# LIU-YUXI/SA-GNN

Hardware: AMD Instinct MI355X
Metric: spmm_edges_per_sec (higher is better)
Workload: dtype f32

## Files before the change

### include/sagnn.h

```cpp
#ifndef SAGNN_H
#define SAGNN_H

#include <stddef.h>
#include <stdint.h>

#ifdef __cplusplus
extern "C" {
#endif

#define SAGNN_VERSION 10400

enum {
  SAGNN_OK = 0,
  SAGNN_ERR_NULL = -1,
  SAGNN_ERR_DIM = -2,
  SAGNN_ERR_ALIGN = -3,
  SAGNN_ERR_CSR = -4,
  SAGNN_ERR_ARG = -5,
  SAGNN_ERR_WORKSPACE = -6,
  SAGNN_ERR_NOMEM = -7
};

int sagnn_version(void);

// ... 93 lines not shown
  const sagnn_spmm_plan* adj_user;
  const sagnn_spmm_plan* adj_item;
  const sagnn_spmm_batch* adj_batch;
  void* adj_workspace;
  size_t adj_workspace_bytes;
} sagnn_edge_time;

int sagnn_spmm_time_batch_create(const sagnn_spmm_plan* const* adj_user, const sagnn_spmm_plan* const* adj_item,
                                 int n_intervals, sagnn_spmm_batch** batch_out);

int sagnn_spmm_time_f32(const sagnn_spmm_plan* plan, const float* X, int64_t ldx, int d,
                        const sagnn_spmm_epilogue* epilogue, const sagnn_edge_drop* drop, const sagnn_edge_time* time,
                        void* workspace, size_t workspace_bytes, void* stream);

typedef struct sagnn_gnn_side {
  const float* in;   int64_t ld_in,  slab_in;
  float*       out;  int64_t ld_out, slab_out;
  float*       scratch;
  uint8_t*     mask;
} sagnn_gnn_side;

enum { SAGNN_EDGES_PLAIN = 0, SAGNN_EDGES_DROP = 1, SAGNN_EDGES_TIME = 2 };

typedef struct sagnn_gnn_args {
  sagnn_gnn_side user, item;
  int d, n_layers;
  float leaky;
  int edges;
  const sagnn_edge_drop* drop;
  const sagnn_edge_time* time;
  int interval;
  void* workspace; size_t workspace_bytes;
} sagnn_gnn_args;

int sagnn_gnn_interval_f32(const sagnn_spmm_plan* plan_user, const sagnn_spmm_plan* plan_item, const sagnn_gnn_args* args,
                           void* stream);
int sagnn_gnn_interval_bwd_f32(const sagnn_spmm_plan* plan_user, const sagnn_spmm_plan* plan_item,
                               const sagnn_gnn_args* args, void* stream);
int sagnn_gnn_stack_f32(const sagnn_spmm_batch* batch, const sagnn_gnn_args* args, void* stream);
int sagnn_gnn_stack_bwd_f32(const sagnn_spmm_batch* batch, const sagnn_gnn_args* args, void* stream);

int sagnn_lstm_fwd_f32(const float* x, int64_t ld_n, int64_t ld_t, int64_t n, int t, int d, const float* W,
                       const float* b, float forget_bias, const float* drop_scale, float* h,
                       int64_t ld_h, void* stream);
int sagnn_lstm_fwd_state_f32(const float* x, int64_t ld_n, int64_t ld_t, int64_t n, int t, int d,
                             const float* W, const float* b, float forget_bias, const float* drop_scale,
                             const float* h_init, int64_t ld_hi, const float* c_init, float* h, int64_t ld_h,
                             float* c_final, void* stream);
int sagnn_layernorm_td_f32(const float* x, int64_t ld_n, int64_t ld_t, int64_t n, int t, int d,
                           const float* gamma, const float* beta, float eps, float* y,
                           int64_t ld_y, void* stream);
int sagnn_mhsa_mean_f32(const float* x, int64_t ld_n, int64_t ld_t, int64_t n, int t, int d, int heads,
                        const float* Wq, const float* bq, const float* Wk, const float* bk,
                        const float* Wv, const float* bv, float* out, int64_t ld_out,
                        void* stream);
size_t sagnn_mhsa_wide_workspace_bytes(int64_t n, int t, int d);
int sagnn_mhsa_mean_wide_f32(const float* x, int64_t ld_n, int64_t ld_t, int64_t n, int t, int d, int heads,
                             const float* Wq, const float* bq, const float* Wk, const float* bk, const float* Wv,
                             const float* bv, float* out, int64_t ld_out, void* workspace, size_t workspace_bytes,
                             void* stream);
size_t sagnn_ln_mhsa_mean_workspace_bytes(int64_t n, int t, int d, int heads);
int sagnn_ln_mhsa_mean_f32(const float* x, int64_t ld_n, int64_t ld_t, int64_t n, int t, int d, int heads,
                           const float* ln_gamma, const float* ln_beta, float ln_eps, const float* Wq,
                           const float* bq, const float* Wk, const float* bk, const float* Wv, const float* bv,
                           float* out, int64_t ld_out, void* workspace, size_t workspace_bytes, void* stream);
int sagnn_interval_fusion_f32(const float* x, int64_t ld_n, int64_t ld_t, int64_t n, int t, int d, int heads,
// ... 160 lines not shown
```

### sa-gnn_amd/_lib.py

```python
from __future__ import annotations

import ctypes
import os
from ctypes import POINTER, c_char_p, c_float, c_int, c_int32, c_int64, c_size_t, c_uint32, c_uint64, c_void_p

_HERE = os.path.dirname(os.path.abspath(__file__))
LIB_PATH = os.environ.get("SAGNN_LIB") or os.path.join(_HERE, "lib", "libsagnn.so")


class SagnnError(RuntimeError):
    def __init__(self, code: int, msg: str):
        super().__init__(f"libsagnn error {code}: {msg}")
        self.code = code


class Tuning(ctypes.Structure):
    _fields_ = [("short_thresh", c_int32), ("long_thresh", c_int32), ("chunk_edges", c_int32),
                ("reserved", c_int32)]


class SpmmEpilogue(ctypes.Structure):
    _fields_ = [("leaky", c_float), ("residual", c_void_p), ("ldr", c_int64), ("out", c_void_p),
                ("ldo", c_int64), ("acc_in", c_void_p), ("ld_acc_in", c_int64), ("acc_out", c_void_p),
                ("ld_acc_out", c_int64), ("mask_out", c_void_p), ("mask_in", c_void_p),
# ... 27 lines not shown

class PlanInfo(ctypes.Structure):
    _fields_ = [("n_rows", c_int64), ("n_src", c_int64), ("nnz", c_int64),
                ("n_long_rows", c_int64), ("n_chunks", c_int64), ("short_thresh", c_int32),
                ("long_thresh", c_int32), ("chunk_edges", c_int32), ("max_degree", c_int32),
                ("on_device", c_int32), ("weighted", c_int32)]


SIGNATURES = {
    "sagnn_version": (c_int, []),
    "sagnn_set_engine": (c_int, [c_int]),
    "sagnn_get_engine": (c_int, []),
    "sagnn_range_redo_count": (c_int, [POINTER(c_int64), c_int]),
    "sagnn_last_error": (c_size_t, [c_char_p, c_size_t]),
    "sagnn_profile_enable": (c_int, [c_int]),
    "sagnn_profile_read": (c_int, [c_void_p, c_void_p, c_void_p, c_void_p, c_int, POINTER(c_int)]),
    "sagnn_csr_check_host": (c_int, [c_void_p, c_void_p, c_int64, c_int64, c_int64]),
    "sagnn_spmm_plan_create": (c_int, [c_void_p, c_void_p, c_void_p, c_int64, c_int64, c_int64,
                                       POINTER(Tuning), POINTER(c_void_p)]),
    "sagnn_spmm_plan_destroy": (c_int, [c_void_p]),
    "sagnn_spmm_plan_get_info": (c_int, [c_void_p, POINTER(PlanInfo)]),
    "sagnn_spmm_plan_set_weights": (c_int, [c_void_p, c_void_p]),
    "sagnn_spmm_plan_copy_chunks": (c_int, [c_void_p, c_void_p, c_void_p, c_void_p, c_int64]),
    "sagnn_spmm_workspace_bytes": (c_size_t, [c_void_p, c_int]),
    "sagnn_spmm_f32": (c_int, [c_void_p, c_void_p, c_int64, c_int, c_void_p, c_int64, c_float,
                               c_void_p, c_int64, c_void_p, c_int64, c_void_p, c_int64, c_void_p,
                               c_size_t, c_void_p]),
    "sagnn_spmm_ex_f32": (c_int, [c_void_p, c_void_p, c_int64, c_int, POINTER(SpmmEpilogue), c_void_p, c_size_t,
                                  c_void_p]),
    "sagnn_mask_scale_f32": (c_int, [c_void_p, c_int64, c_void_p, c_float, c_void_p, c_int64, c_int64, c_int, c_void_p]),
    "sagnn_spmm_batch_create": (c_int, [c_void_p, c_void_p, c_int, POINTER(c_void_p)]),
    "sagnn_spmm_batch_destroy": (c_int, [c_void_p]),
    "sagnn_spmm_batch_workspace_bytes": (c_size_t, [c_void_p, c_int]),
    "sagnn_gnn_interval_f32": (c_int, [c_void_p, c_void_p, POINTER(GnnArgs), c_void_p]),
    "sagnn_gnn_interval_bwd_f32": (c_int, [c_void_p, c_void_p, POINTER(GnnArgs), c_void_p]),
    "sagnn_gnn_stack_f32": (c_int, [c_void_p, POINTER(GnnArgs), c_void_p]),
    "sagnn_gnn_stack_bwd_f32": (c_int, [c_void_p, POINTER(GnnArgs), c_void_p]),
    "sagnn_spmm_drop_f32": (c_int, [c_void_p, c_void_p, c_int64, c_int, POINTER(SpmmEpilogue), POINTER(EdgeDropArgs),
                                    c_uint32, c_int, c_void_p, c_size_t, c_void_p]),
    "sagnn_spmm_plan_set_buckets": (c_int, [c_void_p, c_void_p, c_int32]),
    "sagnn_spmm_time_batch_create": (c_int, [c_void_p, c_void_p, c_int, POINTER(c_void_p)]),
    "sagnn_spmm_time_f32": (c_int, [c_void_p, c_void_p, c_int64, c_int, POINTER(SpmmEpilogue), POINTER(EdgeDropArgs),
                                    POINTER(EdgeTimeArgs), c_void_p, c_size_t, c_void_p]),
    "sagnn_lstm_fwd_train_f32": (c_int, [c_void_p, c_int64, c_int64, c_int64, c_int, c_int, c_void_p, c_void_p, c_float,
                                         c_void_p, c_void_p, c_int64, c_void_p, c_void_p, c_void_p]),
    "sagnn_mhsa_wide_workspace_bytes": (c_size_t, [c_int64, c_int, c_int]),
    "sagnn_ln_mhsa_mean_workspace_bytes": (c_size_t, [c_int64, c_int, c_int, c_int]),
    "sagnn_ln_mhsa_mean_f32": (c_int, [c_void_p, c_int64, c_int64, c_int64, c_int, c_int, c_int, c_void_p, c_void_p,
                                       c_float, c_void_p, c_void_p, c_void_p, c_void_p, c_void_p, c_void_p, c_void_p,
                                       c_int64, c_void_p, c_size_t, c_void_p]),
    "sagnn_mhsa_mean_wide_f32": (c_int, [c_void_p, c_int64, c_int64, c_int64, c_int, c_int, c_int, c_void_p, c_void_p,
                                         c_void_p, c_void_p, c_void_p, c_void_p, c_void_p, c_int64, c_void_p, c_size_t,
                                         c_void_p]),
    "sagnn_attn_bwd_f32": (c_int, [c_void_p, c_void_p, c_int64, c_int64, c_int, c_int, c_int, c_void_p]),
    "sagnn_layernorm_td_bwd_f32": (c_int, [c_void_p, c_int64, c_void_p, c_int64, c_int64, c_int, c_int, c_void_p,
                                           c_float, c_void_p, c_int64, c_void_p, c_void_p, c_void_p]),
    "sagnn_lstm_bwd_step_f32": (c_int, [c_void_p, c_void_p, c_void_p, c_int64, c_void_p, c_void_p, c_int64, c_void_p,
                                        c_void_p, c_void_p, c_int64, c_int, c_int, c_int, c_void_p]),
    "sagnn_attn_bwd_front_supported": (c_int, [c_int, c_int, c_int]),
    "sagnn_attn_bwd_front_f32": (c_int, [c_void_p, c_int64, c_int64, c_int64, c_int, c_int, c_int, c_void_p, c_void_p,
                                         c_float, c_int, c_void_p, c_void_p, c_void_p, c_void_p, c_void_p, c_void_p,
                                         c_void_p, c_int64, c_void_p, c_void_p, c_void_p]),
    "sagnn_attn_bwd_tail_supported": (c_int, [c_int]),
    "sagnn_attn_bwd_tail_f32": (c_int, [c_void_p, c_void_p, c_int64, c_int, c_void_p, c_void_p, c_void_p, c_void_p]),
    "sagnn_lstm_bwd_supported": (c_int, [c_int]),
    "sagnn_lstm_bwd_f32": (c_int, [c_void_p, c_int64, c_int64, c_void_p, c_void_p, c_void_p, c_void_p, c_int64, c_void_p,
# ... 130 lines not shown
```

### sa-gnn_amd/csrc/spmm.hip

```cpp
#include <float.h>

#include <algorithm>
#include <new>
#include <type_traits>
#include <vector>

#include "common.h"
#include "philox.h"

namespace {

constexpr int kWave = 64;
constexpr int kBlock = 256;
constexpr int kWavesPerBlock = kBlock / kWave;
constexpr int kRowsPerWave = 16;
constexpr int64_t kSmallRows = 262144;
constexpr int kUnroll = 8;

struct Epilogue {
  const float* residual;
  int64_t ldr;
  const float* acc_in;
  int64_t ld_acc_in;
  float* out;
// ... 362 lines not shown
          else cw[u] = 1.f;
          if constexpr (TIME) cb[u] = __shfl(bk, grp * LPR + j + u);
          else cb[u] = 0;
        }
#pragma unroll
        for (int u = 0; u < kUnroll; ++u) {
          v[u] = make_float4(0.f, 0.f, 0.f, 0.f);
          if (c[u] >= 0 && lane_on) v[u] = ld4(X + (int64_t)c[u] * ldx + col);
        }
        if constexpr (TIME) {
#pragma unroll
          for (int u = 0; u < kUnroll; ++u)
            if (c[u] >= 0 && lane_on) add4(v[u], ld4(tm.te + cb[u] * d + col));
        }
#pragma unroll
        for (int u = 0; u < kUnroll; ++u) acc4<WEIGHTED>(acc, cw[u], v[u]);
      }
    }
    if (mine && lane_on) finish_row(ep, row0 + lr, col, drop_scale<DROP>(dr, acc));
  }

  while (medium) {
    const int lr = __builtin_ctzll(medium);
    medium &= medium - 1;
    const int e0 = __builtin_amdgcn_readlane(rp, lr);
    const int dg = __builtin_amdgcn_readlane(deg_l, lr);
    const float4 s =
        wave_row_sum<LPR, false, DROP, WEIGHTED, TIME>(colidx, e0, e0 + dg, X, ldx, lane, grp, col, lane_on, dr, (int)row0 + lr, w,
                                                       tm, d);
    if (grp == 0 && lane_on) finish_row(ep, row0 + lr, col, drop_scale<DROP>(dr, s));
  }
}

template <int LPR, int RPW, class... DropArgs>
__global__ __launch_bounds__(kBlock) void spmm_rows_kernel(
    const int32_t* __restrict__ rowptr, const int32_t* __restrict__ colidx,
    const float* __restrict__ X, int64_t ldx, int d, int64_t n_rows, int short_t, int long_t,
    const int32_t* __restrict__ chunk_e0, const int32_t* __restrict__ chunk_e1, int64_t n_chunks,
    int chunk_blocks, float* __restrict__ partial, Epilogue ep, typename KernelArg<DropArgs>::type... da) {
  constexpr bool DROP = Pack<DropArgs...>::DROP, WEIGHTED = Pack<DropArgs...>::WEIGHTED, TIME = Pack<DropArgs...>::TIME;
  const int lane = threadIdx.x & (kWave - 1);
  const int wave = threadIdx.x / kWave;

  if ((int)blockIdx.x < chunk_blocks) {
    const int grp = lane / LPR;
    const int col = 4 * (lane % LPR);
    const bool lane_on = col < d;
    const int64_t ci = (int64_t)blockIdx.x * kWavesPerBlock + wave;
    if (ci >= n_chunks) return;
    const float4 s = wave_row_sum<LPR, false, DROP, WEIGHTED, TIME>(
        colidx, chunk_e0[ci], chunk_e1[ci], X, ldx, lane, grp, col, lane_on, arg_of<RowDrop, DropArgs...>(da...),
        chunk_row_of<DropArgs...>(ci, da...), weights_of<DropArgs...>(0, da...), arg_of<RowTime, DropArgs...>(da...), d);
    if (grp == 0 && lane_on) st4(partial + ci * (int64_t)d + col, s);
    return;
  }

  const int64_t row0 = ((int64_t)(blockIdx.x - chunk_blocks) * kWavesPerBlock + wave) * RPW;
  if (row0 >= n_rows) return;
  rows_wave<LPR, RPW, DROP, WEIGHTED, TIME>(rowptr, colidx, X, ldx, d, n_rows, row0, short_t, long_t, ep, lane,
                                            arg_of<RowDrop, DropArgs...>(da...), weights_of<DropArgs...>(0, da...),
                                            arg_of<RowTime, DropArgs...>(da...));
}

template <int LPR, class... Scale>
__global__ __launch_bounds__(kBlock) void spmm_fixup_kernel(const int32_t* __restrict__ long_row,
                                                           const int32_t* __restrict__ long_slot,
                                                           int64_t n_long,
                                                           const float* __restrict__ partial, int d,
                                                           Epilogue ep, Scale... scale) {
  static_assert(sizeof...(Scale) <= 1, "drop-only argument: none, or the scale");
  const int lane = threadIdx.x & (kWave - 1);
  const int wave = threadIdx.x / kWave;
  const int grp = lane / LPR;
  const int col = 4 * (lane % LPR);
  const bool lane_on = col < d;
  const int64_t li = (int64_t)blockIdx.x * kWavesPerBlock + wave;
  if (li >= n_long) return;
  const float4 s = wave_row_sum<LPR, true>(nullptr, long_slot[li], long_slot[li + 1], partial, d,
                                           lane, grp, col, lane_on);
  if (grp == 0 && lane_on) finish_row(ep, long_row[li], col, scaled(s, scale...));
}

struct SegMeta {
  const int32_t* rowptr;
  const int32_t* colidx;
  int32_t short_t, long_t;
};
struct DirArgs {
  const float* X;
  int64_t ldx, s_X;
  Epilogue ep;
  int64_t s_res, s_acc_in, s_out, s_acc_out, s_mask_out, s_mask_in, s_out2, s_acc_in2;
};
struct BatchGeom {
  int32_t T;
  int32_t chunk_blocks;
  int32_t blocks_u, blocks_i;
  int32_t rows_u, rows_i;
};

__device__ __forceinline__ Epilogue seg_epilogue(const DirArgs& a, int k) {
  Epilogue e = a.ep;
  if (e.residual) e.residual += (int64_t)k * a.s_res;
  if (e.acc_in) e.acc_in += (int64_t)k * a.s_acc_in;
  if (e.out) e.out += (int64_t)k * a.s_out;
  if (e.acc_out) e.acc_out += (int64_t)k * a.s_acc_out;
  if (e.mask_out) e.mask_out += (int64_t)k * a.s_mask_out;
  if (e.mask_in) e.mask_in += (int64_t)k * a.s_mask_in;
  if (e.out2) e.out2 += (int64_t)k * a.s_out2;
  if (e.acc_in2) e.acc_in2 += (int64_t)k * a.s_acc_in2;
  return e;
}

// ... 228 lines not shown
    return sagnn::fail(SAGNN_ERR_ALIGN, "buckets: pointer must be 2-byte aligned");
  plan->d_buckets = d_buckets;
  plan->n_buckets = d_buckets ? n_buckets : 0;
  return SAGNN_OK;
}

extern "C" int sagnn_spmm_plan_get_info(const sagnn_spmm_plan* plan, sagnn_spmm_plan_info* info) {
  if (!plan || !info) return sagnn::fail(SAGNN_ERR_NULL, "plan/info is NULL");
  *info = plan->info;
  return SAGNN_OK;
}

extern "C" int sagnn_spmm_plan_copy_chunks(const sagnn_spmm_plan* plan, int32_t* rows,
                                           int32_t* e_begin, int32_t* e_end, int64_t cap) {
  if (!plan) return sagnn::fail(SAGNN_ERR_NULL, "plan is NULL");
  const int64_t n = plan->info.n_chunks;
  if (cap < n) return sagnn::fail(SAGNN_ERR_ARG, "cap %lld < n_chunks %lld", (long long)cap, (long long)n);
  if (n > 0 && (!rows || !e_begin || !e_end)) return sagnn::fail(SAGNN_ERR_NULL, "null output array");
  std::copy(plan->chunk_row.begin(), plan->chunk_row.end(), rows);
  std::copy(plan->chunk_e0.begin(), plan->chunk_e0.end(), e_begin);
  std::copy(plan->chunk_e1.begin(), plan->chunk_e1.end(), e_end);
  return SAGNN_OK;
}

extern "C" size_t sagnn_spmm_workspace_bytes(const sagnn_spmm_plan* plan, int d) {
  if (!plan || d <= 0) return 0;
  return (size_t)plan->info.n_chunks * (size_t)d * sizeof(float);
}

namespace {

template <int LPR>
int launch_spmm(const sagnn_spmm_plan* p, const float* X, int64_t ldx, int d, const Epilogue& ep,
                float* partial, hipStream_t stream, const RowDrop* drop = nullptr, const float* te = nullptr) {
  const int64_t n_rows = p->info.n_rows;
  const int64_t n_chunks = p->info.n_chunks;
  const int64_t chunk_blocks = (n_chunks + kWavesPerBlock - 1) / kWavesPerBlock;
  constexpr int G = kWave / LPR;
  constexpr int RPW_SMALL = G > 4 ? G : 4;
  const bool small = n_rows < kSmallRows;
  const int64_t rows_per_block = (int64_t)kWavesPerBlock * (small ? RPW_SMALL : kRowsPerWave);
  const int64_t row_blocks = (n_rows + rows_per_block - 1) / rows_per_block;
  const int64_t blocks = chunk_blocks + row_blocks;
  if (blocks > INT32_MAX) return sagnn::fail(SAGNN_ERR_ARG, "grid too large");
  if (blocks > 0) {
    sagnn::ProfileScope prof(sagnn::kProfSpmmRows, stream, p->info.nnz, n_rows);
    const auto rows = [&](auto kernel, auto... da) {
      hipLaunchKernelGGL(kernel, dim3((unsigned)blocks), dim3(kBlock), 0, stream, p->d_rowptr, p->d_colidx, X, ldx, d, n_rows,
                         p->info.short_thresh, p->info.long_thresh, p->d_chunk_e0, p->d_chunk_e1, n_chunks,
                         (int)chunk_blocks, partial, ep, da...);
    };
    const float* w = p->d_weights;
    const RowTime tm{p->d_buckets, te};
    if (te && w)
      rows(small ? spmm_rows_kernel<LPR, RPW_SMALL, RowTime, const float*> : spmm_rows_kernel<LPR, kRowsPerWave, RowTime, const float*>,
           tm, w);
    else if (te)
      rows(small ? spmm_rows_kernel<LPR, RPW_SMALL, RowTime> : spmm_rows_kernel<LPR, kRowsPerWave, RowTime>, tm);
    else if (drop && w)
      rows(small ? spmm_rows_kernel<LPR, RPW_SMALL, const int32_t*, RowDrop, const float*>
                 : spmm_rows_kernel<LPR, kRowsPerWave, const int32_t*, RowDrop, const float*>,
           p->d_chunk_row, *drop, w);
    else if (drop)
      rows(small ? spmm_rows_kernel<LPR, RPW_SMALL, const int32_t*, RowDrop> : spmm_rows_kernel<LPR, kRowsPerWave, const int32_t*, RowDrop>,
           p->d_chunk_row, *drop);
    else if (w)
      rows(small ? spmm_rows_kernel<LPR, RPW_SMALL, const float*> : spmm_rows_kernel<LPR, kRowsPerWave, const float*>, w);
    else
      rows(small ? spmm_rows_kernel<LPR, RPW_SMALL> : spmm_rows_kernel<LPR, kRowsPerWave>);
    SAGNN_HIP_TRY(hipGetLastError());
  }
  const int64_t n_long = p->info.n_long_rows;
  if (n_long > 0) {
    sagnn::ProfileScope prof(sagnn::kProfSpmmFixup, stream, n_chunks, n_long);
    const int64_t fb = (n_long + kWavesPerBlock - 1) / kWavesPerBlock;
    const auto fixup = [&](auto kernel, auto... scale) {
      hipLaunchKernelGGL(kernel, dim3((unsigned)fb), dim3(kBlock), 0, stream,
                         p->d_long_row, p->d_long_slot, n_long, partial, d, ep, scale...);
    };
    if (drop) fixup(spmm_fixup_kernel<LPR, float>, drop->scale);
    else fixup(spmm_fixup_kernel<LPR>);
    SAGNN_HIP_TRY(hipGetLastError());
  }
  return SAGNN_OK;
}

int check_mat(const char* name, const void* ptr, int64_t ld, int d, bool required) {
  if (!ptr) return required ? sagnn::fail(SAGNN_ERR_NULL, "%s is NULL", name) : SAGNN_OK;
  if (!sagnn::aligned16(ptr) || (ld & 3) != 0)
    return sagnn::fail(SAGNN_ERR_ALIGN, "%s: pointer must be 16-byte aligned and ld a multiple of 4", name);
  if (ld < d) return sagnn::fail(SAGNN_ERR_ARG, "%s: ld %lld < d %d", name, (long long)ld, d);
  return SAGNN_OK;
}

int check_d(int d) {
  if (d < 4 || d > 256 || (d & 3)) return sagnn::fail(SAGNN_ERR_DIM, "d = %d: need a multiple of 4 in [4, 256]", d);
  return SAGNN_OK;
}

struct Slab {
  float* p;
  int64_t ld, slab;
};

int check_slab(const char* name, const Slab& x, int d) {
  if (int rc = check_mat(name, x.p, x.ld, d, true)) return rc;
  if (x.slab & 3) return sagnn::fail(SAGNN_ERR_ALIGN, "%s: slab stride must be a multiple of 4", name);
  return SAGNN_OK;
}

int launch_mask_scale(const Slab& g, const uint8_t* mask, int64_t s_mask, float slope, const Slab& out, int64_t n_rows,
                      int d, int64_t T, hipStream_t stream) {
  const int64_t n = n_rows * (d / 4);
  if (n == 0) return SAGNN_OK;
  hipLaunchKernelGGL(mask_scale_kernel, dim3((unsigned)((n + 255) / 256), (unsigned)T), dim3(256), 0, stream, g.p, g.ld,
                     g.slab, mask, s_mask, d / 4, slope, out.p, out.ld, out.slab, n_rows, d);
  SAGNN_HIP_TRY(hipGetLastError());
  return SAGNN_OK;
}

Epilogue kernel_epilogue(const sagnn_spmm_epilogue& e, int d) {
  return Epilogue{e.residual, e.ldr,      e.acc_in,  e.ld_acc_in, e.out,  e.ldo,    e.acc_out, e.ld_acc_out,
                  e.leaky,    e.mask_out, e.mask_in, e.out2,      e.ldo2, e.slope2, d / 4,     e.acc_in2,
                  e.ld_acc_in2};
}

int spmm_ex(const sagnn_spmm_plan* plan, const float* X, int64_t ldx, int d, const Epilogue& e, void* workspace,
            size_t workspace_bytes, void* stream, const RowDrop* drop = nullptr, const float* te = nullptr) {
  if (!plan->info.on_device) return sagnn::fail(SAGNN_ERR_ARG, "plan was built host-only (no device CSR)");
  if (int rc = check_d(d)) return rc;
  if (te) {
    if (drop) return sagnn::fail(SAGNN_ERR_ARG, "edge time: no product takes a drop and a time term");
    if (!plan->d_buckets) return sagnn::fail(SAGNN_ERR_ARG, "edge time: the plan has no buckets (sagnn_spmm_plan_set_buckets)");
    if (!sagnn::aligned16(te)) return sagnn::fail(SAGNN_ERR_ALIGN, "edge time: TE must be 16-byte aligned");
  }
  if (!e.out && !e.acc_out && !e.out2) return sagnn::fail(SAGNN_ERR_NULL, "no output given");
  if (int rc = check_mat("X", X, ldx, d, plan->info.nnz > 0)) return rc;
  if (int rc = check_mat("residual", e.residual, e.ldr, d, false)) return rc;
  if (int rc = check_mat("out", e.out, e.ldo, d, false)) return rc;
  if (int rc = check_mat("acc_in", e.acc_in, e.ld_acc_in, d, false)) return rc;
  if (int rc = check_mat("acc_out", e.acc_out, e.ld_acc_out, d, false)) return rc;
  if (int rc = check_mat("acc_in2", e.acc_in2, e.ld_acc_in2, d, false)) return rc;
  if (e.acc_in2 && !e.acc_out) return sagnn::fail(SAGNN_ERR_ARG, "acc_in2 given without acc_out");
  if (int rc = check_mat("out2", e.out2, e.ldo2, d, false)) return rc;
  if ((e.out && e.out == X) || (e.acc_out && e.acc_out == X) || (e.out2 && e.out2 == X))
    return sagnn::fail(SAGNN_ERR_ARG, "outputs must not alias X");
  if (e.mask_in && !e.out2) return sagnn::fail(SAGNN_ERR_ARG, "mask_in given without out2");
  const size_t need = sagnn_spmm_workspace_bytes(plan, d);
  if (need > 0) {
    if (!workspace || workspace_bytes < need)
      return sagnn::fail(SAGNN_ERR_WORKSPACE, "workspace needs %zu bytes, got %zu", need,
                         workspace ? workspace_bytes : (size_t)0);
    if (!sagnn::aligned16(workspace)) return sagnn::fail(SAGNN_ERR_ALIGN, "workspace not 16-byte aligned");
  }
  if (plan->info.n_rows == 0) return SAGNN_OK;

  hipStream_t s = static_cast<hipStream_t>(stream);
  float* partial = static_cast<float*>(workspace);
  switch (sagnn::lanes_per_row(d)) {
    case 8: return launch_spmm<8>(plan, X, ldx, d, e, partial, s, drop, te);
    case 16: return launch_spmm<16>(plan, X, ldx, d, e, partial, s, drop, te);
    case 32: return launch_spmm<32>(plan, X, ldx, d, e, partial, s, drop, te);
    default: return launch_spmm<64>(plan, X, ldx, d, e, partial, s, drop, te);
  }
}

}

extern "C" int sagnn_spmm_ex_f32(const sagnn_spmm_plan* plan, const float* X, int64_t ldx, int d,
                                 const sagnn_spmm_epilogue* e, void* workspace, size_t workspace_bytes,
                                 void* stream) {
  if (!plan || !e) return sagnn::fail(SAGNN_ERR_NULL, "plan/epilogue is NULL");
  return spmm_ex(plan, X, ldx, d, kernel_epilogue(*e, d), workspace, workspace_bytes, stream);
}

namespace {
constexpr int kDropMaxLayers = 127;
constexpr int64_t kDropMaxIntervals = 1 << 23;

int check_drop(const sagnn_edge_drop* drop, int n_layers, int64_t last_interval) {
  if (!drop) return sagnn::fail(SAGNN_ERR_NULL, "edge drop: the sagnn_edge_drop is NULL");
  if (drop->keep_threshold == 0) return sagnn::fail(SAGNN_ERR_ARG, "edge drop: keep_threshold = 0 keeps no edge");
  if (!(drop->scale > 0.f) || !(drop->scale <= FLT_MAX))
    return sagnn::fail(SAGNN_ERR_ARG, "edge drop: scale = %g, need a finite value > 0", (double)drop->scale);
  if (n_layers > kDropMaxLayers)
    return sagnn::fail(SAGNN_ERR_ARG, "edge drop: n_layers = %d, the tag holds %d", n_layers, kDropMaxLayers);
  if (last_interval < 0 || last_interval >= kDropMaxIntervals)
    return sagnn::fail(SAGNN_ERR_ARG, "edge drop: interval %lld outside [0, 2^23)", (long long)last_interval);
  return SAGNN_OK;
}

RowDrop row_drop(const sagnn_edge_drop& e, uint32_t tag, bool rows_users) {
  return RowDrop{(uint32_t)e.seed, (uint32_t)(e.seed >> 32), e.step, e.keep_threshold, tag, rows_users ? 1 : 0, e.scale};
}
}

extern "C" int sagnn_spmm_drop_f32(const sagnn_spmm_plan* plan, const float* X, int64_t ldx, int d,
// ... 368 lines not shown
  int operator()(int, const Slab&, const Slab&) const { return SAGNN_OK; }
};
template <class Launch, class BeforeStep = NoBeforeStep>
int run_backward(const Stack& st, Launch launch, void* stream, BeforeStep before_step = BeforeStep{}) {
  for (const Side* s : {&st.u, &st.i}) {
    const int64_t mrow = st.d / 4;
    if (int rc = launch_mask_scale(s->in, s->mask + (int64_t)(st.n_layers - 1) * s->rows * mrow, st.n_layers * s->rows * mrow,
                                   st.leaky, scratch_slot(st, *s, 2), s->rows, st.d, st.T, static_cast<hipStream_t>(stream)))
      return rc;
  }
  for (int l = st.n_layers - 1; l >= 0; --l) {
    const int cur = (st.n_layers - 1 - l) & 1;
    if (int rc = before_step(l, scratch_slot(st, st.u, 2 + cur), scratch_slot(st, st.i, 2 + cur))) return rc;
    if (int rc = launch(backward_step(st, st.u, st.i, l), backward_step(st, st.i, st.u, l),
                        LayerTags{(uint32_t)l << 1 | 1u, (uint32_t)l << 1, l}))
      return rc;
  }
  return SAGNN_OK;
}

auto batched(const sagnn_spmm_batch* b, int d, void* workspace, void* stream) {
  return [=](const DirArgs& au, const DirArgs& ai, const LayerTags&) {
    return launch_batch_d(b, d, au, ai, static_cast<float*>(workspace), static_cast<hipStream_t>(stream));
  };
}

auto batched_drop(const sagnn_spmm_batch* b, int d, void* workspace, void* stream, const sagnn_edge_drop& drop) {
  return [=](const DirArgs& au, const DirArgs& ai, const LayerTags& t) {
    const BatchDrop bd{row_drop(drop, t.tag_u, true), t.tag_i};
    return launch_batch_d(b, d, au, ai, static_cast<float*>(workspace), static_cast<hipStream_t>(stream), &bd);
  };
}

auto per_plan(const sagnn_spmm_plan* plan_user, const sagnn_spmm_plan* plan_item, int d, void* workspace,
              size_t workspace_bytes, void* stream) {
  return [=](const DirArgs& au, const DirArgs& ai, const LayerTags&) {
    if (int rc = spmm_ex(plan_user, au.X, au.ldx, d, au.ep, workspace, workspace_bytes, stream)) return rc;
    return spmm_ex(plan_item, ai.X, ai.ldx, d, ai.ep, workspace, workspace_bytes, stream);
  };
}

auto per_plan_drop(const sagnn_spmm_plan* plan_user, const sagnn_spmm_plan* plan_item, int d, void* workspace,
                   size_t workspace_bytes, void* stream, const sagnn_edge_drop& drop, int interval) {
  return [=](const DirArgs& au, const DirArgs& ai, const LayerTags& t) {
    const uint32_t k = (uint32_t)interval << 8;
    const RowDrop du = row_drop(drop, t.tag_u | k, true), di = row_drop(drop, t.tag_i | k, false);
    if (int rc = spmm_ex(plan_user, au.X, au.ldx, d, au.ep, workspace, workspace_bytes, stream, &du)) return rc;
    return spmm_ex(plan_item, ai.X, ai.ldx, d, ai.ep, workspace, workspace_bytes, stream, &di);
  };
}

int check_time(const sagnn_edge_time* t, const sagnn_edge_drop* drop, int32_t n_buckets, int d) {
  if (drop) return sagnn::fail(SAGNN_ERR_ARG, "edge time: edge dropout and time do not combine (drop must be NULL)");
  if (!t || !t->te) return sagnn::fail(SAGNN_ERR_NULL, "edge time: the sagnn_edge_time or its te is NULL");
  if (n_buckets == 0) return sagnn::fail(SAGNN_ERR_ARG, "edge time: the plans carry no buckets (sagnn_spmm_plan_set_buckets)");
  if (t->n_buckets != n_buckets)
    return sagnn::fail(SAGNN_ERR_ARG, "edge time: n_buckets = %d but the plans were given %d", t->n_buckets, n_buckets);
  if (!sagnn::aligned16(t->te) || ((t->stride_interval | t->stride_layer | t->stride_dir) & 3) || (d & 3))
    return sagnn::fail(SAGNN_ERR_ALIGN, "edge time: te must be 16-byte aligned and its strides multiples of 4");
  return SAGNN_OK;
}

int check_time_bwd(const sagnn_edge_time* t, bool stack, int64_t U, int64_t I, int T) {
  if (!t->dte) return sagnn::fail(SAGNN_ERR_NULL, "edge time: dte is NULL");
  if (!sagnn::aligned16(t->dte)) return sagnn::fail(SAGNN_ERR_ALIGN, "edge time: dte must be 16-byte aligned");
  if (stack) {
    const sagnn_spmm_batch* b = t->adj_batch;
    if (!b) return sagnn::fail(SAGNN_ERR_NULL, "edge time: adj_batch is NULL");
    if (b->T != T || b->U != t->n_buckets || b->I != t->n_buckets)
      return sagnn::fail(SAGNN_ERR_ARG, "edge time: adj_batch is not the time batch of %d intervals and %d buckets", T, t->n_buckets);
    return SAGNN_OK;
// ... 120 lines not shown
  if (int rc = check_form(g, a, false)) return rc;
  if (int rc = check_graphs(g)) return rc;
  const sagnn_gnn_side &u = a->user, &i = a->item;
  if (!u.in || !i.in || !u.out || !i.out) return sagnn::fail(SAGNN_ERR_NULL, "null embedding pointer");
  if (g.stack)
    if (int rc = check_d(a->d)) return rc;
  if (a->n_layers < 1) return sagnn::fail(SAGNN_ERR_ARG, "n_layers = %d: need >= 1", a->n_layers);
  if ((u.mask == nullptr) != (i.mask == nullptr)) return sagnn::fail(SAGNN_ERR_NULL, "give both masks or neither");
  if (a->n_layers > 1 && (!u.scratch || !i.scratch))
    return sagnn::fail(SAGNN_ERR_NULL, "scratch buffers required for n_layers > 1");
  if (!g.stack) {
    if (!g.plan_user->info.on_device) return sagnn::fail(SAGNN_ERR_ARG, "plan was built host-only (no device CSR)");
    if (int rc = check_d(a->d)) return rc;
  }
  const Stack st = make_stack(g, *a);
  if (int rc = check_stack(st, a->n_layers > 1, "u0", "i0", "user_out", "item_out")) return rc;
  if (g.stack)
    if (int rc = check_batch_ws(g.batch, a->d, a->workspace, a->workspace_bytes)) return rc;
  return with_launcher(g, *a, stream, [&](auto launch) { return run_forward(st, launch); });
}

int gnn_backward(const Graphs& g, const sagnn_gnn_args* a, void* stream) {
  if (int rc = check_form(g, a, true)) return rc;
  if (int rc = check_graphs(g)) return rc;
  const sagnn_gnn_side &u = a->user, &i = a->item;
  if (!u.in || !i.in || !u.out || !i.out || !u.mask || !i.mask || !u.scratch || !i.scratch)
    return sagnn::fail(SAGNN_ERR_NULL, "null pointer");
  if (a->n_layers < 1) return sagnn::fail(SAGNN_ERR_ARG, "n_layers = %d: need >= 1", a->n_layers);
  if (int rc = check_d(a->d)) return rc;
  const Stack st = make_stack(g, *a);
  if (int rc = check_stack(st, true, "G_u", "G_i", "grad_u0", "grad_i0")) return rc;
  if (g.stack)
    if (int rc = check_batch_ws(g.batch, a->d, a->workspace, a->workspace_bytes)) return rc;
  if (a->edges != SAGNN_EDGES_TIME)
    return with_launcher(g, *a, stream, [&](auto launch) { return run_backward(st, launch, stream); });
  const sagnn_edge_time& tm = *a->time;
  if (!g.stack)
    return run_backward(st, per_plan(g.plan_user, g.plan_item, a->d, a->workspace, a->workspace_bytes, stream), stream,
                        dte_per_plan(tm, a->d, a->interval, stream));
  if (int rc = check_batch_ws(tm.adj_batch, a->d, tm.adj_workspace, tm.adj_workspace_bytes)) return rc;
  return run_backward(st, batched(g.batch, a->d, a->workspace, stream), stream, dte_batched(tm, a->d, stream));
}
}

extern "C" int sagnn_gnn_interval_f32(const sagnn_spmm_plan* plan_user, const sagnn_spmm_plan* plan_item,
                                      const sagnn_gnn_args* args, void* stream) {
  return gnn_forward(Graphs{plan_user, plan_item, nullptr, false}, args, stream);
}

extern "C" int sagnn_gnn_interval_bwd_f32(const sagnn_spmm_plan* plan_user, const sagnn_spmm_plan* plan_item,
                                          const sagnn_gnn_args* args, void* stream) {
  return gnn_backward(Graphs{plan_user, plan_item, nullptr, false}, args, stream);
}

extern "C" int sagnn_gnn_stack_f32(const sagnn_spmm_batch* batch, const sagnn_gnn_args* args, void* stream) {
  return gnn_forward(Graphs{nullptr, nullptr, batch, true}, args, stream);
}

extern "C" int sagnn_gnn_stack_bwd_f32(const sagnn_spmm_batch* batch, const sagnn_gnn_args* args, void* stream) {
  return gnn_backward(Graphs{nullptr, nullptr, batch, true}, args, stream);
}

extern "C" int sagnn_spmm_time_f32(const sagnn_spmm_plan* plan, const float* X, int64_t ldx, int d,
                                   const sagnn_spmm_epilogue* e, const sagnn_edge_drop* drop, const sagnn_edge_time* time,
                                   void* workspace, size_t workspace_bytes, void* stream) {
  if (!plan || !e) return sagnn::fail(SAGNN_ERR_NULL, "plan/epilogue is NULL");
  if (int rc = check_time(time, drop, plan->n_buckets, d)) return rc;
  return spmm_ex(plan, X, ldx, d, kernel_epilogue(*e, d), workspace, workspace_bytes, stream, nullptr, time->te);
}
```

### sa-gnn_amd/ops.py

```python
from __future__ import annotations

import ctypes
import math

import numpy as np
import torch

from . import _lib
from ._lib import PlanInfo, Tuning, check

SUPPORTED_D = tuple(range(4, 257, 4))

ENGINES = {"f16x2": 0, "f32": 1, "valu": 2}


def set_engine(name: str) -> None:
    check(_lib.load().sagnn_set_engine(ENGINES[name]))


def get_engine() -> str:
    code = _lib.load().sagnn_get_engine()
    return next(k for k, v in ENGINES.items() if v == code)


# ... 122 lines not shown
        w_t = None if weights is None else _check_weights(weights, self.nnz)
        if w_t is not None and device is None:
            raise ValueError("weights: a host-only plan (device=None) takes no weights")
        if (buckets is None) != (n_buckets is None):
            raise ValueError("buckets: give buckets and n_buckets together")
        b_t = None if buckets is None else _check_buckets(buckets, n_buckets, self.nnz)
        if b_t is not None and device is None:
            raise ValueError("buckets: a host-only plan (device=None) takes no buckets")
        rp_h = rp_t.cpu().contiguous()
        self._rowptr_host = rp_h.numpy()
        if validate:
            ci_h = ci_t.cpu().contiguous()
            check(lib.sagnn_csr_check_host(rp_h.data_ptr(), ci_h.data_ptr(), self.n_rows, self.n_src,
                                           self.nnz))
        tun = None
        if tuning is not None:
            tun = Tuning(int(tuning[0]), int(tuning[1]), int(tuning[2]), 0)
        if device is None:
            self.rowptr = self.colidx = None
            d_rp = d_ci = None
        else:
            self.rowptr = rp_t.to(device).contiguous()
            self.colidx = ci_t.to(device).contiguous()
            if self.colidx.numel() == 0:
                self.colidx = torch.zeros(1, dtype=torch.int32, device=device)
            d_rp, d_ci = self.rowptr.data_ptr(), self.colidx.data_ptr()
        check(lib.sagnn_spmm_plan_create(rp_h.data_ptr(), d_rp, d_ci, self.n_rows, self.n_src,
                                         self.nnz, ctypes.byref(tun) if tun else None,
                                         ctypes.byref(self._h)))
        info = PlanInfo()
        check(lib.sagnn_spmm_plan_get_info(self._h, ctypes.byref(info)))
        self.info = info
        self.device = device
        self._ws: dict[int, torch.Tensor] = {}
        self.partner_adjoint: SpmmPlan | None = None
        self.weights = None
        if w_t is not None:
            self.weights = w_t.to(device).contiguous()
            if self.weights.numel() == 0:
                self.weights = torch.zeros(1, dtype=torch.float32, device=device)
            check(lib.sagnn_spmm_plan_set_weights(self._h, self.weights.data_ptr()))
            check(lib.sagnn_spmm_plan_get_info(self._h, ctypes.byref(info)))
        self.buckets, self.n_buckets = None, 0
        self._tuning = tuning
        self._time_adjoint: SpmmPlan | None = None
        if b_t is not None:
            self._buckets_host = b_t.numpy()
            self._weights_host = None if w_t is None else w_t.numpy()
            self.n_buckets = int(n_buckets)
            self.buckets = b_t.to(device).contiguous()
            if self.buckets.numel() == 0:
                self.buckets = torch.zeros(1, dtype=torch.uint16, device=device)
            check(lib.sagnn_spmm_plan_set_buckets(self._h, self.buckets.data_ptr(), self.n_buckets))

    @property
    def time_adjoint(self) -> "SpmmPlan":
        if self.buckets is None:
            raise ValueError("time_adjoint: the plan has no buckets")
        if self._time_adjoint is None:
            rp, ci, w = time_adjoint_arrays(self._rowptr_host, self._buckets_host, self.n_buckets, self._weights_host)
            self._time_adjoint = SpmmPlan(rp, ci, self.n_buckets, self.n_rows, device=self.device, tuning=self._tuning,
                                          validate=False, weights=w)
        return self._time_adjoint

    @property
    def weighted(self) -> bool:
        return self.weights is not None
# ... 143 lines not shown
        a.stride_layer = te.stride(-4)
        a.stride_interval = te.stride(0) if stack else 0
        self.keep = [te, dte, adj]
        if dte is not None:
            a.dte = dte.data_ptr()
            if stack:
                a.adj_batch = adj.handle
                ws = adj.workspace(d)
            else:
                a.adj_user, a.adj_item = adj[0].handle, adj[1].handle
                ws = _interval_ws(adj[0], adj[1], d)
            self.keep.append(ws)
            a.adj_workspace, a.adj_workspace_bytes = _ptr(ws), 0 if ws is None else ws.numel() * 4
        self.args = a


def spmm_time(plan: SpmmPlan, x: torch.Tensor | None, leaky: float, te: torch.Tensor, residual=None, out=None, acc_in=None,
              acc_out=None, acc_in2=None, mask_out=None, mask_in=None, out2=None, slope2: float = 1.0,
              want_out: bool = False):
    if plan.buckets is None:
        raise ValueError("spmm_time: the plan has no buckets (SpmmPlan(..., buckets=, n_buckets=))")
    return spmm_ex(plan, x, leaky, residual, out, acc_in, acc_out, acc_in2, mask_out, mask_in, out2, slope2, want_out,
                   _time=te)


def mask_scale(g: torch.Tensor, mask: torch.Tensor, slope: float, out: torch.Tensor):
    rows, d = int(g.shape[0]), int(g.shape[1])
    _masks("mask", mask, (rows, d // 4))
    check(_lib.load().sagnn_mask_scale_f32(_ptr(g), _f32_rows("g", g, d, rows), _ptr(mask), float(slope), _ptr(out),
                                           _f32_rows("out", out, d, rows), rows, d, _stream()))
    return out


def _interval_ws(plan_user: SpmmPlan, plan_item: SpmmPlan, d: int):
    wu, wi = plan_user.workspace(d), plan_item.workspace(d)
    return wu if (wi is None or (wu is not None and wu.numel() >= wi.numel())) else wi


def _scratch(name: str, s: torch.Tensor | None, k: int, rows: int, d: int, device):
    if s is None:
        return torch.empty(k * rows * d, dtype=torch.float32, device=device)
    if s.dtype != torch.float32 or not s.is_contiguous() or s.numel() < k * rows * d:
        raise ValueError(f"{name}: need a contiguous float32 buffer of {k}*{rows}*{d} elements")
    return s


def _masks(name: str, m: torch.Tensor, shape: tuple):
    if m.dtype != torch.uint8 or not m.is_contiguous() or m.numel() != int(np.prod(shape)):
        raise ValueError(f"{name}: need a contiguous uint8 tensor {list(shape)}")
    return m


def _adjoint_pair(plan_user: SpmmPlan, plan_item: SpmmPlan):
    adj_u, adj_i = plan_user.partner_adjoint, plan_item.partner_adjoint
    if (adj_u is None) != (adj_i is None):
        raise ValueError("give the exact adjoint of both plans or of neither")
    if adj_u is not None:
        return adj_u, adj_i
    if plan_user.nnz != plan_item.nnz:
        raise ValueError(f"plans are not a transposed pair (nnz {plan_user.nnz} vs {plan_item.nnz}: duplicated stored "
                         "entries?) — build them with graph.interval_pair, which adds the exact adjoints")
    return plan_user, plan_item


def _gnn_args(user: tuple, item: tuple, d: int, n_layers: int, leaky: float, drop, interval: int, et, ws):
    if et is not None and drop is not None:
        raise ValueError("edge dropout and time do not combine: give `drop` or `time`, not both")
    a = _lib.GnnArgs()
    for side, (x, ld_in, slab_in, out, ld_out, slab_out, scratch, mask) in ((a.user, user), (a.item, item)):
# ... 1186 lines not shown
```

Before: 17.65 billion.

## Fold first side's long-row fixup into second side's SpMM launch

In the interval GNN forward, the two per-side SpMM calls now use separate workspace regions. The long-row fixup of the first side runs as extra guest blocks at the front of the second side's rows kernel instead of as its own launch. This removes one kernel launch and its serialization per layer, and orders the side with more chunks first. The cost is a larger combined workspace, a new workspace check, and a dispatch branch at the start of every plain SpMM kernel block.

```diff
diff --git a/include/sagnn.h b/include/sagnn.h
--- a/include/sagnn.h
+++ b/include/sagnn.h
@@ -149,6 +149,9 @@
   int interval;
   void* workspace; size_t workspace_bytes;
 } sagnn_gnn_args;
+
+size_t sagnn_gnn_interval_workspace_bytes(const sagnn_spmm_plan* plan_user, const sagnn_spmm_plan* plan_item, int d);
+int sagnn_gnn_interval_first_side(const sagnn_spmm_plan* plan_user, const sagnn_spmm_plan* plan_item);
 
 int sagnn_gnn_interval_f32(const sagnn_spmm_plan* plan_user, const sagnn_spmm_plan* plan_item, const sagnn_gnn_args* args,
                            void* stream);
diff --git a/sa-gnn_amd/_lib.py b/sa-gnn_amd/_lib.py
--- a/sa-gnn_amd/_lib.py
+++ b/sa-gnn_amd/_lib.py
@@ -83,6 +83,8 @@
     "sagnn_spmm_batch_create": (c_int, [c_void_p, c_void_p, c_int, POINTER(c_void_p)]),
     "sagnn_spmm_batch_destroy": (c_int, [c_void_p]),
     "sagnn_spmm_batch_workspace_bytes": (c_size_t, [c_void_p, c_int]),
+    "sagnn_gnn_interval_workspace_bytes": (c_size_t, [c_void_p, c_void_p, c_int]),
+    "sagnn_gnn_interval_first_side": (c_int, [c_void_p, c_void_p]),
     "sagnn_gnn_interval_f32": (c_int, [c_void_p, c_void_p, POINTER(GnnArgs), c_void_p]),
     "sagnn_gnn_interval_bwd_f32": (c_int, [c_void_p, c_void_p, POINTER(GnnArgs), c_void_p]),
     "sagnn_gnn_stack_f32": (c_int, [c_void_p, POINTER(GnnArgs), c_void_p]),
diff --git a/sa-gnn_amd/csrc/spmm.hip b/sa-gnn_amd/csrc/spmm.hip
--- a/sa-gnn_amd/csrc/spmm.hip
+++ b/sa-gnn_amd/csrc/spmm.hip
@@ -418,21 +418,56 @@
   }
 }
 
+template <int LPR, class... Scale>
+__device__ __forceinline__ void fixup_wave(const int32_t* __restrict__ long_row, const int32_t* __restrict__ long_slot,
+                                           int64_t n_long, const float* __restrict__ partial, int d, const Epilogue& ep,
+                                           int block, Scale... scale) {
+  static_assert(sizeof...(Scale) <= 1, "drop-only argument: none, or the scale");
+  const int lane = threadIdx.x & (kWave - 1);
+  const int wave = threadIdx.x / kWave;
+  const int grp = lane / LPR;
+  const int col = 4 * (lane % LPR);
+  const bool lane_on = col < d;
+  const int64_t li = (int64_t)block * kWavesPerBlock + wave;
+  if (li >= n_long) return;
+  const float4 s = wave_row_sum<LPR, true>(nullptr, long_slot[li], long_slot[li + 1], partial, d,
+                                           lane, grp, col, lane_on);
+  if (grp == 0 && lane_on) finish_row(ep, long_row[li], col, scaled(s, scale...));
+}
+
+struct Guest {
+  const int32_t* long_row;
+  const int32_t* long_slot;
+  const float* partial;
+  int64_t n_long;
+  int blocks;
+  int d;
+  Epilogue ep;
+};
+
 template <int LPR, int RPW, class... DropArgs>
 __global__ __launch_bounds__(kBlock) void spmm_rows_kernel(
     const int32_t* __restrict__ rowptr, const int32_t* __restrict__ colidx,
     const float* __restrict__ X, int64_t ldx, int d, int64_t n_rows, int short_t, int long_t,
     const int32_t* __restrict__ chunk_e0, const int32_t* __restrict__ chunk_e1, int64_t n_chunks,
-    int chunk_blocks, float* __restrict__ partial, Epilogue ep, typename KernelArg<DropArgs>::type... da) {
+    int chunk_blocks, float* __restrict__ partial, Epilogue ep, Guest guest, typename KernelArg<DropArgs>::type... da) {
   constexpr bool DROP = Pack<DropArgs...>::DROP, WEIGHTED = Pack<DropArgs...>::WEIGHTED, TIME = Pack<DropArgs...>::TIME;
+  int block = (int)blockIdx.x;
+  if constexpr (!DROP && !TIME) {
+    if (block < guest.blocks) {
+      fixup_wave<LPR>(guest.long_row, guest.long_slot, guest.n_long, guest.partial, guest.d, guest.ep, block);
+      return;
+    }
+    block -= guest.blocks;
+  }
   const int lane = threadIdx.x & (kWave - 1);
   const int wave = threadIdx.x / kWave;
 
-  if ((int)blockIdx.x < chunk_blocks) {
+  if (block < chunk_blocks) {
     const int grp = lane / LPR;
     const int col = 4 * (lane % LPR);
     const bool lane_on = col < d;
-    const int64_t ci = (int64_t)blockIdx.x * kWavesPerBlock + wave;
+    const int64_t ci = (int64_t)block * kWavesPerBlock + wave;
     if (ci >= n_chunks) return;
     const float4 s = wave_row_sum<LPR, false, DROP, WEIGHTED, TIME>(
         colidx, chunk_e0[ci], chunk_e1[ci], X, ldx, lane, grp, col, lane_on, arg_of<RowDrop, DropArgs...>(da...),
@@ -441,7 +476,7 @@
     return;
   }
 
-  const int64_t row0 = ((int64_t)(blockIdx.x - chunk_blocks) * kWavesPerBlock + wave) * RPW;
+  const int64_t row0 = ((int64_t)(block - chunk_blocks) * kWavesPerBlock + wave) * RPW;
   if (row0 >= n_rows) return;
   rows_wave<LPR, RPW, DROP, WEIGHTED, TIME>(rowptr, colidx, X, ldx, d, n_rows, row0, short_t, long_t, ep, lane,
                                             arg_of<RowDrop, DropArgs...>(da...), weights_of<DropArgs...>(0, da...),
@@ -454,17 +489,7 @@
                                                            int64_t n_long,
                                                            const float* __restrict__ partial, int d,
                                                            Epilogue ep, Scale... scale) {
-  static_assert(sizeof...(Scale) <= 1, "drop-only argument: none, or the scale");
-  const int lane = threadIdx.x & (kWave - 1);
-  const int wave = threadIdx.x / kWave;
-  const int grp = lane / LPR;
-  const int col = 4 * (lane % LPR);
-  const bool lane_on = col < d;
-  const int64_t li = (int64_t)blockIdx.x * kWavesPerBlock + wave;
-  if (li >= n_long) return;
-  const float4 s = wave_row_sum<LPR, true>(nullptr, long_slot[li], long_slot[li + 1], partial, d,
-                                           lane, grp, col, lane_on);
-  if (grp == 0 && lane_on) finish_row(ep, long_row[li], col, scaled(s, scale...));
+  fixup_wave<LPR>(long_row, long_slot, n_long, partial, d, ep, (int)blockIdx.x, scale...);
 }
 
 struct SegMeta {
@@ -759,7 +784,8 @@
 
 template <int LPR>
 int launch_spmm(const sagnn_spmm_plan* p, const float* X, int64_t ldx, int d, const Epilogue& ep,
-                float* partial, hipStream_t stream, const RowDrop* drop = nullptr, const float* te = nullptr) {
+                float* partial, hipStream_t stream, const RowDrop* drop = nullptr, const float* te = nullptr,
+                const Guest* guest = nullptr, bool own_fixup = true) {
   const int64_t n_rows = p->info.n_rows;
   const int64_t n_chunks = p->info.n_chunks;
   const int64_t chunk_blocks = (n_chunks + kWavesPerBlock - 1) / kWavesPerBlock;
@@ -768,14 +794,16 @@
   const bool small = n_rows < kSmallRows;
   const int64_t rows_per_block = (int64_t)kWavesPerBlock * (small ? RPW_SMALL : kRowsPerWave);
   const int64_t row_blocks = (n_rows + rows_per_block - 1) / rows_per_block;
-  const int64_t blocks = chunk_blocks + row_blocks;
+  if (guest && (drop || te)) return sagnn::fail(SAGNN_ERR_ARG, "a drop or time launch carries no guest fix-up");
+  const Guest gst = guest ? *guest : Guest{};
+  const int64_t blocks = gst.blocks + chunk_blocks + row_blocks;
   if (blocks > INT32_MAX) return sagnn::fail(SAGNN_ERR_ARG, "grid too large");
   if (blocks > 0) {
     sagnn::ProfileScope prof(sagnn::kProfSpmmRows, stream, p->info.nnz, n_rows);
     const auto rows = [&](auto kernel, auto... da) {
       hipLaunchKernelGGL(kernel, dim3((unsigned)blocks), dim3(kBlock), 0, stream, p->d_rowptr, p->d_colidx, X, ldx, d, n_rows,
                          p->info.short_thresh, p->info.long_thresh, p->d_chunk_e0, p->d_chunk_e1, n_chunks,
-                         (int)chunk_blocks, partial, ep, da...);
+                         (int)chunk_blocks, partial, ep, gst, da...);
     };
     const float* w = p->d_weights;
     const RowTime tm{p->d_buckets, te};
@@ -798,7 +826,7 @@
     SAGNN_HIP_TRY(hipGetLastError());
   }
   const int64_t n_long = p->info.n_long_rows;
-  if (n_long > 0) {
+  if (n_long > 0 && own_fixup) {
     sagnn::ProfileScope prof(sagnn::kProfSpmmFixup, stream, n_chunks, n_long);
     const int64_t fb = (n_long + kWavesPerBlock - 1) / kWavesPerBlock;
     const auto fixup = [&](auto kernel, auto... scale) {
@@ -852,8 +880,8 @@
                   e.ld_acc_in2};
 }
 
-int spmm_ex(const sagnn_spmm_plan* plan, const float* X, int64_t ldx, int d, const Epilogue& e, void* workspace,
-            size_t workspace_bytes, void* stream, const RowDrop* drop = nullptr, const float* te = nullptr) {
+int spmm_check(const sagnn_spmm_plan* plan, const float* X, int64_t ldx, int d, const Epilogue& e, const void* workspace,
+               size_t workspace_bytes, const RowDrop* drop = nullptr, const float* te = nullptr) {
   if (!plan->info.on_device) return sagnn::fail(SAGNN_ERR_ARG, "plan was built host-only (no device CSR)");
   if (int rc = check_d(d)) return rc;
   if (te) {
@@ -880,16 +908,27 @@
                          workspace ? workspace_bytes : (size_t)0);
     if (!sagnn::aligned16(workspace)) return sagnn::fail(SAGNN_ERR_ALIGN, "workspace not 16-byte aligned");
   }
+  return SAGNN_OK;
+}
+
+int spmm_launch(const sagnn_spmm_plan* plan, const float* X, int64_t ldx, int d, const Epilogue& e, void* workspace,
+                void* stream, const RowDrop* drop = nullptr, const float* te = nullptr, const Guest* guest = nullptr,
+                bool own_fixup = true) {
   if (plan->info.n_rows == 0) return SAGNN_OK;
-
   hipStream_t s = static_cast<hipStream_t>(stream);
   float* partial = static_cast<float*>(workspace);
   switch (sagnn::lanes_per_row(d)) {
-    case 8: return launch_spmm<8>(plan, X, ldx, d, e, partial, s, drop, te);
-    case 16: return launch_spmm<16>(plan, X, ldx, d, e, partial, s, drop, te);
-    case 32: return launch_spmm<32>(plan, X, ldx, d, e, partial, s, drop, te);
-    default: return launch_spmm<64>(plan, X, ldx, d, e, partial, s, drop, te);
-  }
+    case 8: return launch_spmm<8>(plan, X, ldx, d, e, partial, s, drop, te, guest, own_fixup);
+    case 16: return launch_spmm<16>(plan, X, ldx, d, e, partial, s, drop, te, guest, own_fixup);
+    case 32: return launch_spmm<32>(plan, X, ldx, d, e, partial, s, drop, te, guest, own_fixup);
+    default: return launch_spmm<64>(plan, X, ldx, d, e, partial, s, drop, te, guest, own_fixup);
+  }
+}
+
+int spmm_ex(const sagnn_spmm_plan* plan, const float* X, int64_t ldx, int d, const Epilogue& e, void* workspace,
+            size_t workspace_bytes, void* stream, const RowDrop* drop = nullptr, const float* te = nullptr) {
+  if (int rc = spmm_check(plan, X, ldx, d, e, workspace, workspace_bytes, drop, te)) return rc;
+  return spmm_launch(plan, X, ldx, d, e, workspace, stream, drop, te);
 }
 
 }
@@ -1324,11 +1363,29 @@
   };
 }
 
+bool item_side_first(const sagnn_spmm_plan* plan_user, const sagnn_spmm_plan* plan_item) {
+  return plan_item->info.n_chunks > plan_user->info.n_chunks;
+}
+
 auto per_plan(const sagnn_spmm_plan* plan_user, const sagnn_spmm_plan* plan_item, int d, void* workspace,
               size_t workspace_bytes, void* stream) {
   return [=](const DirArgs& au, const DirArgs& ai, const LayerTags&) {
-    if (int rc = spmm_ex(plan_user, au.X, au.ldx, d, au.ep, workspace, workspace_bytes, stream)) return rc;
-    return spmm_ex(plan_item, ai.X, ai.ldx, d, ai.ep, workspace, workspace_bytes, stream);
+    const size_t need_u = sagnn_spmm_workspace_bytes(plan_user, d);
+    char* const ws_u = static_cast<char*>(workspace);
+    char* const ws_i = ws_u ? ws_u + need_u : nullptr;
+    const size_t bytes_i = workspace_bytes > need_u ? workspace_bytes - need_u : 0;
+    const bool swap = item_side_first(plan_user, plan_item);
+    const sagnn_spmm_plan *p1 = swap ? plan_item : plan_user, *p2 = swap ? plan_user : plan_item;
+    const DirArgs &a1 = swap ? ai : au, &a2 = swap ? au : ai;
+    char *const ws1 = swap ? ws_i : ws_u, *const ws2 = swap ? ws_u : ws_i;
+    if (int rc = spmm_check(p1, a1.X, a1.ldx, d, a1.ep, ws1, swap ? bytes_i : workspace_bytes)) return rc;
+    if (int rc = spmm_check(p2, a2.X, a2.ldx, d, a2.ep, ws2, swap ? workspace_bytes : bytes_i)) return rc;
+    const int64_t n_long = p1->info.n_long_rows;
+    const bool carry = n_long > 0 && p1->info.n_rows > 0 && p2->info.n_rows > 0;
+    const Guest guest{p1->d_long_row, p1->d_long_slot, reinterpret_cast<const float*>(ws1), n_long,
+                      (int)((n_long + kWavesPerBlock - 1) / kWavesPerBlock), d, a1.ep};
+    if (int rc = spmm_launch(p1, a1.X, a1.ldx, d, a1.ep, ws1, stream, nullptr, nullptr, nullptr, !carry)) return rc;
+    return spmm_launch(p2, a2.X, a2.ldx, d, a2.ep, ws2, stream, nullptr, nullptr, carry ? &guest : nullptr);
   };
 }
 
@@ -1515,6 +1572,11 @@
   if (int rc = check_stack(st, true, "G_u", "G_i", "grad_u0", "grad_i0")) return rc;
   if (g.stack)
     if (int rc = check_batch_ws(g.batch, a->d, a->workspace, a->workspace_bytes)) return rc;
+  if (!g.stack && a->edges != SAGNN_EDGES_DROP && g.plan_user->info.on_device && g.plan_item->info.on_device) {
+    const size_t need = sagnn_gnn_interval_workspace_bytes(g.plan_user, g.plan_item, a->d);
+    if (need > 0 && (!a->workspace || a->workspace_bytes < need))
+      return sagnn::fail(SAGNN_ERR_WORKSPACE, "workspace needs %zu bytes, got %zu", need, a->workspace ? a->workspace_bytes : (size_t)0);
+  }
   if (a->edges != SAGNN_EDGES_TIME)
     return with_launcher(g, *a, stream, [&](auto launch) { return run_backward(st, launch, stream); });
   const sagnn_edge_time& tm = *a->time;
@@ -1526,6 +1588,15 @@
 }
 }
 
+extern "C" size_t sagnn_gnn_interval_workspace_bytes(const sagnn_spmm_plan* plan_user, const sagnn_spmm_plan* plan_item, int d) {
+  return sagnn_spmm_workspace_bytes(plan_user, d) + sagnn_spmm_workspace_bytes(plan_item, d);
+}
+
+extern "C" int sagnn_gnn_interval_first_side(const sagnn_spmm_plan* plan_user, const sagnn_spmm_plan* plan_item) {
+  if (!plan_user || !plan_item) return sagnn::fail(SAGNN_ERR_NULL, "plan is NULL");
+  return item_side_first(plan_user, plan_item) ? 1 : 0;
+}
+
 extern "C" int sagnn_gnn_interval_f32(const sagnn_spmm_plan* plan_user, const sagnn_spmm_plan* plan_item,
                                       const sagnn_gnn_args* args, void* stream) {
   return gnn_forward(Graphs{plan_user, plan_item, nullptr, false}, args, stream);
diff --git a/sa-gnn_amd/ops.py b/sa-gnn_amd/ops.py
--- a/sa-gnn_amd/ops.py
+++ b/sa-gnn_amd/ops.py
@@ -178,7 +178,7 @@
         check(lib.sagnn_spmm_plan_get_info(self._h, ctypes.byref(info)))
         self.info = info
         self.device = device
-        self._ws: dict[int, torch.Tensor] = {}
+        self._ws: dict = {}
         self.partner_adjoint: SpmmPlan | None = None
         self.weights = None
         if w_t is not None:
@@ -388,9 +388,26 @@
     return out
 
 
+def interval_workspace_bytes(plan_user: SpmmPlan, plan_item: SpmmPlan, d: int) -> int:
+    return int(plan_user._lib.sagnn_gnn_interval_workspace_bytes(plan_user.handle, plan_item.handle, int(d)))
+
+
+def interval_first_side(plan_user: SpmmPlan, plan_item: SpmmPlan) -> int:
+    side = int(plan_user._lib.sagnn_gnn_interval_first_side(plan_user.handle, plan_item.handle))
+    check(min(side, 0))
+    return side
+
+
 def _interval_ws(plan_user: SpmmPlan, plan_item: SpmmPlan, d: int):
-    wu, wi = plan_user.workspace(d), plan_item.workspace(d)
-    return wu if (wi is None or (wu is not None and wu.numel() >= wi.numel())) else wi
+    need = interval_workspace_bytes(plan_user, plan_item, d)
+    if need == 0:
+        return None
+    key = ("pair", id(plan_item), d)
+    held = plan_user._ws.get(key)
+    if held is None or held[0] is not plan_item or held[1].numel() * 4 < need:
+        held = (plan_item, torch.empty(need // 4, dtype=torch.float32, device=plan_user.device))
+        plan_user._ws[key] = held
+    return held[1]
 
 
 def _scratch(name: str, s: torch.Tensor | None, k: int, rows: int, d: int, device):
```

Result: no change. 17.64 billion (-0.0%).
